# tdunnlab/scrubvae

Hardware: AMD Instinct MI355X
Metric: pose-windows/sec (ELBO-match) on synthetic 64-frame mouse skeletons (higher is better)
Workload: dtype f32 (f16x3b3 split on the fp16 / bf16 matrix cores); 1 GPU; configs[2] full SC-VAE (conditional + grad_reversal x2 + adversarial_net), AdamW, batch 4096/GPU, window 64, 23 joints, z=32, channels [64,128,256,512,1024]; batch_per_gpu=4096, global_batch=4096, window=64, joints=23, launch=eager launches, inputs=resident in HBM, side_streams=2, parallelism=dp1, backend=none, ranks_seen=1, bn=single rank

## Files before the change

scrubvae_amd/csrc/pose_tail.hip:

```cpp
#include "svae_internal.h"
#include <cstdlib>

namespace svae {

struct TailArgs {
  const float* y;
  const float* offsets;
  const float* target;
  const float* root;
  const float* ext_dx6d;
  const float* ext_droot;
  float* x6d_hat;
  float* root_hat;
  float* loss_part;
  float* dy;
  float* pose_out;
  long long rows;
  int ld, J, ldt, ldo;
  int has_arena;
  int pre_tanh;
  float a0[3], a1[3];
  float jpe_scale, root_scale;
  svae_tree tree;
};

struct M3 {
  float m[9];
};

__device__ __forceinline__ M3 mul(const M3& a, const M3& b) {
  M3 c;
#pragma unroll
  for (int r = 0; r < 3; ++r)
#pragma unroll
    for (int k = 0; k < 3; ++k) c.m[r * 3 + k] = a.m[r * 3] * b.m[k] + a.m[r * 3 + 1] * b.m[3 + k] + a.m[r * 3 + 2] * b.m[6 + k];
  return c;
}
__device__ __forceinline__ M3 mul_tn(const M3& a, const M3& b) {
  M3 c;
#pragma unroll
  for (int r = 0; r < 3; ++r)
#pragma unroll
    for (int k = 0; k < 3; ++k) c.m[r * 3 + k] = a.m[r] * b.m[k] + a.m[3 + r] * b.m[3 + k] + a.m[6 + r] * b.m[6 + k];
  return c;
}
__device__ __forceinline__ M3 mul_nt(const M3& a, const M3& b) {
  M3 c;
#pragma unroll
  for (int r = 0; r < 3; ++r)
#pragma unroll
    for (int k = 0; k < 3; ++k)
      c.m[r * 3 + k] = a.m[r * 3] * b.m[k * 3] + a.m[r * 3 + 1] * b.m[k * 3 + 1] + a.m[r * 3 + 2] * b.m[k * 3 + 2];
  return c;
}

__device__ __forceinline__ void cross3(const float* a, const float* b, float* c) {
  c[0] = a[1] * b[2] - a[2] * b[1];
  c[1] = a[2] * b[0] - a[0] * b[2];
  c[2] = a[0] * b[1] - a[1] * b[0];
}

constexpr float K1_EPS = 1e-8f;

__device__ __forceinline__ M3 c6_to_mat(const float* a) {
  const float nx = sqrtf(a[0] * a[0] + a[1] * a[1] + a[2] * a[2]);
  const float ix = 1.f / (nx + K1_EPS);
  const float x[3] = {a[0] * ix, a[1] * ix, a[2] * ix};
  float zr[3];
  cross3(x, a + 3, zr);
  const float nz = sqrtf(zr[0] * zr[0] + zr[1] * zr[1] + zr[2] * zr[2]);
  const float iz = 1.f / (nz + K1_EPS);
  const float z[3] = {zr[0] * iz, zr[1] * iz, zr[2] * iz};
  float yv[3];
  cross3(z, x, yv);
  M3 M;
#pragma unroll
  for (int r = 0; r < 3; ++r) { M.m[r * 3] = x[r]; M.m[r * 3 + 1] = yv[r]; M.m[r * 3 + 2] = z[r]; }
  return M;
}

__device__ __forceinline__ void c6_to_mat_bwd(const float* a, const M3& dM, float* da) {
  const float nx = sqrtf(a[0] * a[0] + a[1] * a[1] + a[2] * a[2]);
  const float ix = 1.f / (nx + K1_EPS);
  const float x[3] = {a[0] * ix, a[1] * ix, a[2] * ix};
  float zr[3];
  cross3(x, a + 3, zr);
  const float nz = sqrtf(zr[0] * zr[0] + zr[1] * zr[1] + zr[2] * zr[2]);
  const float iz = 1.f / (nz + K1_EPS);
  const float z[3] = {zr[0] * iz, zr[1] * iz, zr[2] * iz};
  float gx[3] = {dM.m[0], dM.m[3], dM.m[6]}, gy[3] = {dM.m[1], dM.m[4], dM.m[7]}, gz[3] = {dM.m[2], dM.m[5], dM.m[8]};
  float t[3];
  cross3(x, gy, t);
  gz[0] += t[0]; gz[1] += t[1]; gz[2] += t[2];
  cross3(gy, z, t);
  gx[0] += t[0]; gx[1] += t[1]; gx[2] += t[2];
  const float dzr_dot = zr[0] * gz[0] + zr[1] * gz[1] + zr[2] * gz[2];
  const float kz = nz > 0.f ? dzr_dot * iz * iz / nz : 0.f;
  const float gzr[3] = {gz[0] * iz - zr[0] * kz, gz[1] * iz - zr[1] * kz, gz[2] * iz - zr[2] * kz};
  cross3(a + 3, gzr, t);
  gx[0] += t[0]; gx[1] += t[1]; gx[2] += t[2];
  cross3(gzr, x, da + 3);
  const float dx_dot = a[0] * gx[0] + a[1] * gx[1] + a[2] * gx[2];
  const float kx = nx > 0.f ? dx_dot * ix * ix / nx : 0.f;
  da[0] = gx[0] * ix - a[0] * kx;
  da[1] = gx[1] * ix - a[1] * kx;
  da[2] = gx[2] * ix - a[2] * kx;
}

template <int TR>
__global__ __launch_bounds__(64 * SVAE_MAX_CHAINS) void pose_tail_kernel(const TailArgs g) {
  extern __shared__ __attribute__((aligned(16))) float smem[];
  const int tid = threadIdx.x, nth = blockDim.x;
  const int wave = tid >> 6, lane = tid & 63;
  const int J = g.J, J3 = 3 * J, C6 = 6 * J;
  const int ldt = g.ldt, ldo = g.ldo;
  float* tile = smem;
  float* offs = tile + TR * ldt;
  float* pose = offs + TR * ldo;
  float* dm0 = pose + TR * ldo;
  float* red = dm0 + TR * 9;
  const long long r0 = (long long)blockIdx.x * TR;
  const int nrows = (int)((g.rows - r0) < TR ? (g.rows - r0) : TR);
  const int n_chains = g.tree.n_chains;

  {
    const int f4_per_row = g.ld / 4;
    const int total = nrows * f4_per_row;
    const float* src = g.y + r0 * g.ld;
    for (int e = tid; e < total; e += nth) {
      const int rr = e / f4_per_row, c = (e - rr * f4_per_row) * 4;
      const float4 v = *reinterpret_cast<const float4*>(src + (long long)e * 4);
      float* d = tile + rr * ldt + c;
      if (g.pre_tanh) { d[0] = tanhf(v.x); d[1] = tanhf(v.y); d[2] = tanhf(v.z); d[3] = tanhf(v.w); }
      else { d[0] = v.x; d[1] = v.y; d[2] = v.z; d[3] = v.w; }
    }
    const int tot3 = nrows * J3;
    const float* so = g.offsets + r0 * J3;
    for (int e = tid; e < tot3; e += nth) {
      const int rr = e / J3, c = e - rr * J3;
      offs[rr * ldo + c] = so[e];
    }
    for (int e = tid; e < TR * 9; e += nth) dm0[e] = 0.f;
  }
  __syncthreads();
  {
    const int tot6 = nrows * C6;
    float* dst = g.x6d_hat + r0 * C6;
    for (int e = tid; e < tot6; e += nth) {
      const int rr = e / C6, c = e - rr * C6;
      dst[e] = tile[rr * ldt + c];
    }
    if (g.has_arena) {
      float* dr = g.root_hat + r0 * 3;
      for (int e = tid; e < nrows * 3; e += nth) {
        const int rr = e / 3, k = e - rr * 3;
        dr[e] = 0.5f * (tile[rr * ldt + C6 + k] + 1.f) * (g.a1[k] - g.a0[k]) + g.a0[k];
      }
    }
  }

  const bool active = lane < nrows;
  const int lrow = lane < TR ? lane : 0;
  float* my = tile + lrow * ldt;
  float* myo = offs + lrow * ldo;
  float* myp = pose + lrow * ldo;
  const bool do_bwd = g.dy != nullptr;
  const bool chain_wave = wave < n_chains && g.tree.chain_len[wave < n_chains ? wave : 0] >= 2;
  const int ch = wave < n_chains ? wave : 0;
  const int len = g.tree.chain_len[ch];

  float a6[6];
  M3 M0;
  if (active) {
#pragma unroll
    for (int k = 0; k < 6; ++k) a6[k] = my[k];
    M0 = c6_to_mat(a6);
  }
  M3 Rc = M0;
  if (active && chain_wave) {
    M3& R = Rc;
    float acc[3] = {0.f, 0.f, 0.f};
    for (int i = 1; i < len; ++i) {
      const int j = g.tree.chain[ch][i];
#pragma unroll
      for (int k = 0; k < 6; ++k) a6[k] = my[6 * j + k];
      R = mul(R, c6_to_mat(a6));
      const float o0 = myo[3 * j], o1 = myo[3 * j + 1], o2 = myo[3 * j + 2];
#pragma unroll
      for (int r = 0; r < 3; ++r) {
        acc[r] += R.m[r * 3] * o0 + R.m[r * 3 + 1] * o1 + R.m[r * 3 + 2] * o2;
        myp[3 * j + r] = acc[r];
      }
    }
  }
  __syncthreads();

  float rl = 0.f;
  if (wave == 0 && active) {
    myp[0] = 0.f; myp[1] = 0.f; myp[2] = 0.f;
    for (int c = 0; c < n_chains; ++c) {
      const int cl = g.tree.chain_len[c];
      const int head = g.tree.chain[c][0];
      const float h0 = myp[3 * head], h1 = myp[3 * head + 1], h2 = myp[3 * head + 2];
      for (int i = 1; i < cl; ++i) {
        const int j = g.tree.chain[c][i];
        myp[3 * j] += h0; myp[3 * j + 1] += h1; myp[3 * j + 2] += h2;
      }
    }
  }
  const int root_wave = nth > 64 ? 1 : 0;
  if (wave == root_wave && active && g.has_arena) {
#pragma unroll
    for (int k = 0; k < 3; ++k) {
      const float xh = my[C6 + k];
      const float half = 0.5f * (g.a1[k] - g.a0[k]);
      const float rh = (xh + 1.f) * half + g.a0[k];
      const float d = rh - g.root[(r0 + lane) * 3 + k];
      rl += d * d;
      if (do_bwd) {
        float gk = 2.f * g.root_scale * d;
        if (g.ext_droot) gk += g.ext_droot[(r0 + lane) * 3 + k];
        my[C6 + k] = g.pre_tanh ? gk * half * (1.f - xh * xh) : gk * half;
      }
    }
  }
  if (wave == root_wave && active && do_bwd) {
    for (int c = C6 + (g.has_arena ? 3 : 0); c < g.ld; ++c) my[c] = 0.f;
  }
  __syncthreads();

  {
    float jpe = 0.f;
    const int tot3 = nrows * J3;
    const float* stg = g.target + r0 * J3;
    float* dp = g.pose_out ? g.pose_out + r0 * J3 : nullptr;
    for (int e = tid; e < tot3; e += nth) {
      const int rr = e / J3, c = e - rr * J3;
      const float pv = pose[rr * ldo + c];
      if (dp) dp[e] = pv;
      const float d = pv - stg[e];
      jpe += d * d;
      pose[rr * ldo + c] = 2.f * g.jpe_scale * d;
    }
    jpe = wave_sum(jpe);
    if (lane == 0) red[wave] = jpe;
  }
  __syncthreads();
  if (tid == 0) {
    float t = 0.f;
    for (int w = 0; w < nth / 64; ++w) t += red[w];
    g.loss_part[blockIdx.x * 2] = t;
  }
  if (do_bwd && wave == 0 && active) {
    for (int c = n_chains - 1; c >= 0; --c) {
      const int cl = g.tree.chain_len[c];
      for (int i = cl - 1; i >= 1; --i) {
        const int j = g.tree.chain[c][i], par = g.tree.chain[c][i - 1];
#pragma unroll
        for (int r = 0; r < 3; ++r) myp[3 * par + r] += myp[3 * j + r];
      }
    }
  }
  if (do_bwd) __syncthreads();

  M3 carry;
#pragma unroll
  for (int k = 0; k < 9; ++k) carry.m[k] = 0.f;
  if (do_bwd && active && chain_wave) {
    M3 P = Rc;
#pragma unroll
    for (int i = SVAE_MAX_CHAIN_LEN - 1; i >= 1; --i) {
      if (i < len) {
        const int j = g.tree.chain[ch][i];
        M3 D = carry;
#pragma unroll
        for (int r = 0; r < 3; ++r)
#pragma unroll
          for (int k = 0; k < 3; ++k) D.m[r * 3 + k] += myp[3 * j + r] * myo[3 * j + k];
#pragma unroll
        for (int k = 0; k < 6; ++k) a6[k] = my[6 * j + k];
        const M3 Mj = c6_to_mat(a6);
        {
          float inv[3];
#pragma unroll
          for (int c = 0; c < 3; ++c) inv[c] = 1.f / (Mj.m[c] * Mj.m[c] + Mj.m[3 + c] * Mj.m[3 + c] + Mj.m[6 + c] * Mj.m[6 + c]);
          M3 Q;
#pragma unroll
          for (int r = 0; r < 3; ++r)
#pragma unroll
            for (int k = 0; k < 3; ++k)
              Q.m[r * 3 + k] = P.m[r * 3] * inv[0] * Mj.m[k * 3] + P.m[r * 3 + 1] * inv[1] * Mj.m[k * 3 + 1] + P.m[r * 3 + 2] * inv[2] * Mj.m[k * 3 + 2];
          P = Q;
        }
        const M3 dMj = mul_tn(P, D);
        carry = mul_nt(D, Mj);
        float da[6];
        c6_to_mat_bwd(a6, dMj, da);
#pragma unroll
        for (int k = 0; k < 6; ++k) {
          float gk = da[k];
          if (g.ext_dx6d) gk += g.ext_dx6d[(r0 + lane) * C6 + 6 * j + k];
          my[6 * j + k] = g.pre_tanh ? gk * (1.f - a6[k] * a6[k]) : gk;
        }
      }
    }
  }
  if (do_bwd) {
    for (int c = 0; c < n_chains; ++c) {
      if (wave == c && chain_wave && active) {
        float* d = dm0 + lane * 9;
#pragma unroll
        for (int k = 0; k < 9; ++k) d[k] += carry.m[k];
      }
      __syncthreads();
    }
  }
  if (do_bwd && wave == 0 && active) {
    M3 dM0;
    const float* d = dm0 + lane * 9;
#pragma unroll
    for (int k = 0; k < 9; ++k) dM0.m[k] = d[k];
    float a0[6], da0[6];
#pragma unroll
    for (int k = 0; k < 6; ++k) a0[k] = my[k];
    c6_to_mat_bwd(a0, dM0, da0);
#pragma unroll
    for (int k = 0; k < 6; ++k) {
      float gk = da0[k];
      if (g.ext_dx6d) gk += g.ext_dx6d[(r0 + lane) * C6 + k];
      my[k] = g.pre_tanh ? gk * (1.f - a0[k] * a0[k]) : gk;
    }
  }
  if (wave == root_wave) {
    rl = wave_sum(rl);
    if (lane == 0) g.loss_part[blockIdx.x * 2 + 1] = rl;
  }
  __syncthreads();
  if (do_bwd) {
    const int f4_per_row = g.ld / 4;
    const int total = nrows * f4_per_row;
    float* dst = g.dy + r0 * g.ld;
    for (int e = tid; e < total; e += nth) {
      const int rr = e / f4_per_row, c = (e - rr * f4_per_row) * 4;
      const float* sp = tile + rr * ldt + c;
      *reinterpret_cast<float4*>(dst + (long long)e * 4) = make_float4(sp[0], sp[1], sp[2], sp[3]);
    }
  }
}

__device__ __forceinline__ void rot6d_rows(const float* d6, float* m ) {
  const float n1 = fmaxf(sqrtf(d6[0] * d6[0] + d6[1] * d6[1] + d6[2] * d6[2]), 1e-12f);
  const float b1[3] = {d6[0] / n1, d6[1] / n1, d6[2] / n1};
  const float dt = b1[0] * d6[3] + b1[1] * d6[4] + b1[2] * d6[5];
  const float u[3] = {d6[3] - dt * b1[0], d6[4] - dt * b1[1], d6[5] - dt * b1[2]};
  const float n2 = fmaxf(sqrtf(u[0] * u[0] + u[1] * u[1] + u[2] * u[2]), 1e-12f);
  const float b2[3] = {u[0] / n2, u[1] / n2, u[2] / n2};
  float b3[3];
  cross3(b1, b2, b3);
#pragma unroll
  for (int k = 0; k < 3; ++k) { m[k] = b1[k]; m[3 + k] = b2[k]; m[6 + k] = b3[k]; }
}

__device__ __forceinline__ void rot6d_rows_bwd(const float* d6, const float* g, float* dd) {
  const float n1r = sqrtf(d6[0] * d6[0] + d6[1] * d6[1] + d6[2] * d6[2]);
  const float n1 = fmaxf(n1r, 1e-12f);
  const float b1[3] = {d6[0] / n1, d6[1] / n1, d6[2] / n1};
  const float dt = b1[0] * d6[3] + b1[1] * d6[4] + b1[2] * d6[5];
  const float u[3] = {d6[3] - dt * b1[0], d6[4] - dt * b1[1], d6[5] - dt * b1[2]};
  const float n2r = sqrtf(u[0] * u[0] + u[1] * u[1] + u[2] * u[2]);
  const float n2 = fmaxf(n2r, 1e-12f);
  const float b2[3] = {u[0] / n2, u[1] / n2, u[2] / n2};
  float gb1[3] = {g[0], g[1], g[2]}, gb2[3] = {g[3], g[4], g[5]};
  const float gb3[3] = {g[6], g[7], g[8]};
  float t[3];
  cross3(b2, gb3, t);
  gb1[0] += t[0]; gb1[1] += t[1]; gb1[2] += t[2];
  cross3(gb3, b1, t);
  gb2[0] += t[0]; gb2[1] += t[1]; gb2[2] += t[2];
  float gu[3];
  if (n2r > 1e-12f) {
    const float d = b2[0] * gb2[0] + b2[1] * gb2[1] + b2[2] * gb2[2];
#pragma unroll
    for (int k = 0; k < 3; ++k) gu[k] = (gb2[k] - b2[k] * d) / n2;
  } else {
#pragma unroll
    for (int k = 0; k < 3; ++k) gu[k] = gb2[k] / n2;
  }
  const float gub1 = gu[0] * b1[0] + gu[1] * b1[1] + gu[2] * b1[2];
#pragma unroll
  for (int k = 0; k < 3; ++k) {
    dd[3 + k] = gu[k] - gub1 * b1[k];
    gb1[k] += -dt * gu[k] - gub1 * d6[3 + k];
  }
  if (n1r > 1e-12f) {
    const float d = b1[0] * gb1[0] + b1[1] * gb1[1] + b1[2] * gb1[2];
#pragma unroll
    for (int k = 0; k < 3; ++k) dd[k] = (gb1[k] - b1[k] * d) / n1;
  } else {
#pragma unroll
    for (int k = 0; k < 3; ++k) dd[k] = gb1[k] / n1;
  }
}

__global__ __launch_bounds__(256) void rot_loss_kernel(const float* __restrict__ x, const float* __restrict__ xh, float scale,
                                                        float* __restrict__ part, float* __restrict__ dxh, long long n) {
  __shared__ float red4[4];
  const long long i = (long long)blockIdx.x * 256 + threadIdx.x;
  float loss = 0.f;
  if (i < n) {
    float a[6], b[6], m1[9], m2[9];
#pragma unroll
    for (int k = 0; k < 6; ++k) { a[k] = x[i * 6 + k]; b[k] = xh[i * 6 + k]; }
    rot6d_rows(a, m1);
    rot6d_rows(b, m2);
    float ss = 0.f, d[9];
#pragma unroll
    for (int k = 0; k < 9; ++k) { d[k] = m2[k] - m1[k]; ss += d[k] * d[k]; }
    const float fro = sqrtf(ss);
    const float c = 0.35355339059327373f;
    float s = fro * c;
    const float lim = 1.f - 1e-7f;
    const bool clamped = s > lim;
    if (clamped) s = lim;
    loss = 2.f * asinf(s);
    if (dxh) {
      float gm[9];
      const float gs = (!clamped && fro > 0.f) ? scale * 2.f / sqrtf(1.f - s * s) * c / fro : 0.f;
#pragma unroll
      for (int k = 0; k < 9; ++k) gm[k] = gs * d[k];
      float dd[6];
      rot6d_rows_bwd(b, gm, dd);
#pragma unroll
      for (int k = 0; k < 6; ++k) dxh[i * 6 + k] = dd[k];
    }
  }
  const float t = block_sum_256(loss, red4);
  if (threadIdx.x == 0) part[blockIdx.x] = t;
}

}

using namespace svae;

static int tail_rows() {
  static int tr = 0;
  if (tr == 0) {
    const char* e = getenv("SVAE_TAIL_ROWS");
    const int v = e ? atoi(e) : 64;
    tr = (v == 64 || v == 48 || v == 32) ? v : 64;
  }
  return tr;
}

extern "C" int svae_tail_blocks(long long rows) { const int tr = tail_rows(); return (int)((rows + tr - 1) / tr); }

extern "C" int svae_pose_tail(const float* y, int ld, const float* offsets, const float* target_pose, const float* root,
                              const float* arena_host, const svae_tree* tree, float jpe_scale, float root_scale,
                              const float* ext_dx6d, const float* ext_droot, float* x6d_hat, float* root_hat, float* loss_part,
                              float* dy, float* pose_out, long long rows, int input_is_pre_tanh, void* stream) {
  SVAE_REQUIRE(y && offsets && target_pose && tree && x6d_hat && loss_part && rows > 0, SVAE_ERR_ARG, "pose_tail: null pointer");
  const int J = tree->n_joints;
  SVAE_REQUIRE(J >= 1 && J <= SVAE_MAX_JOINTS && tree->n_chains >= 0 && tree->n_chains <= SVAE_MAX_CHAINS, SVAE_ERR_SHAPE,
               "pose_tail: bad tree");
  SVAE_REQUIRE(ld % 4 == 0 && ld >= 6 * J + (arena_host ? 3 : 0) && aligned16(y) && (!dy || aligned16(dy)), SVAE_ERR_ALIGN,
               "pose_tail: ld %d too small or misaligned", ld);
  SVAE_REQUIRE(!arena_host || (root && root_hat), SVAE_ERR_ARG, "pose_tail: arena without root buffers");
  int seen[SVAE_MAX_JOINTS] = {0};
  seen[0] = 1;
  for (int c = 0; c < tree->n_chains; ++c) {
    const int len = tree->chain_len[c];
    SVAE_REQUIRE(len >= 1 && len <= SVAE_MAX_CHAIN_LEN, SVAE_ERR_SHAPE, "pose_tail: chain %d length %d", c, len);
    for (int i = 0; i < len; ++i) SVAE_REQUIRE(tree->chain[c][i] >= 0 && tree->chain[c][i] < J, SVAE_ERR_SHAPE, "pose_tail: joint id");
    SVAE_REQUIRE(seen[tree->chain[c][0]], SVAE_ERR_SHAPE, "pose_tail: chain %d starts at a joint not yet placed", c);
    for (int i = 1; i < len; ++i) {
      SVAE_REQUIRE(!seen[tree->chain[c][i]], SVAE_ERR_SHAPE, "pose_tail: joint %d placed twice", tree->chain[c][i]);
      seen[tree->chain[c][i]] = 1;
    }
  }
  for (int j = 0; j < J; ++j) SVAE_REQUIRE(seen[j], SVAE_ERR_SHAPE, "pose_tail: joint %d not covered by the kinematic tree", j);
  TailArgs g;
  memset(&g, 0, sizeof(g));
  g.y = y; g.offsets = offsets; g.target = target_pose; g.root = root; g.ext_dx6d = ext_dx6d; g.ext_droot = ext_droot;
  g.x6d_hat = x6d_hat; g.root_hat = root_hat; g.loss_part = loss_part; g.dy = dy; g.pose_out = pose_out;
  g.rows = rows; g.ld = ld; g.J = J;
  g.ldt = ld | 1;
  g.ldo = (3 * J) | 1;
  g.has_arena = arena_host != nullptr;
  g.pre_tanh = input_is_pre_tanh;
  if (arena_host)
    for (int k = 0; k < 3; ++k) { g.a0[k] = arena_host[k]; g.a1[k] = arena_host[3 + k]; }
  g.jpe_scale = jpe_scale; g.root_scale = root_scale;
  g.tree = *tree;
  const int n_waves = tree->n_chains >= 2 ? tree->n_chains : 2;
  const int tr = tail_rows();
  const size_t smem = (size_t)(tr * g.ldt + 2 * tr * g.ldo + tr * 9 + SVAE_MAX_CHAINS) * sizeof(float);
  SVAE_REQUIRE(smem <= 160 * 1024, SVAE_ERR_SHAPE, "pose_tail: LDS tile %zu B exceeds 160 KiB", smem);
  static DeviceOnce attr_set;
  int attr_dev;
  if (attr_set.need(&attr_dev)) {
    hipError_t e = hipFuncSetAttribute((const void*)pose_tail_kernel<64>, hipFuncAttributeMaxDynamicSharedMemorySize, 160 * 1024);
    if (e == hipSuccess) e = hipFuncSetAttribute((const void*)pose_tail_kernel<48>, hipFuncAttributeMaxDynamicSharedMemorySize, 160 * 1024);
    if (e == hipSuccess) e = hipFuncSetAttribute((const void*)pose_tail_kernel<32>, hipFuncAttributeMaxDynamicSharedMemorySize, 160 * 1024);
    SVAE_REQUIRE(e == hipSuccess, SVAE_ERR_LAUNCH, "pose_tail: hipFuncSetAttribute(MaxDynamicSharedMemorySize): %s", hipGetErrorString(e));
    attr_set.done(attr_dev);
  }
  const dim3 grid(svae_tail_blocks(rows)), block(64 * n_waves);
  if (tr == 64) hipLaunchKernelGGL(pose_tail_kernel<64>, grid, block, smem, (hipStream_t)stream, g);
  else if (tr == 48) hipLaunchKernelGGL(pose_tail_kernel<48>, grid, block, smem, (hipStream_t)stream, g);
  else hipLaunchKernelGGL(pose_tail_kernel<32>, grid, block, smem, (hipStream_t)stream, g);
  return check_launch("pose_tail");
}

extern "C" int svae_rot_blocks(long long n) { return (int)((n + 255) / 256); }

extern "C" int svae_rot_loss(const float* x6d, const float* x6d_hat, float scale, float* part, float* dx6d_hat, long long n,
                             void* stream) {
  SVAE_REQUIRE(x6d && x6d_hat && part && n > 0, SVAE_ERR_ARG, "rot_loss: bad args");
  hipLaunchKernelGGL(rot_loss_kernel, dim3(svae_rot_blocks(n)), dim3(256), 0, (hipStream_t)stream, x6d, x6d_hat, scale, part,
                     dx6d_hat, n);
  return check_launch("rot_loss");
}
```

Before: 293,700 windows/s.

## Restructure pose tail kernel: precompute rotations, parallelize tree passes across threads

Rewrites the forward-kinematics tail so every thread in a larger block (up to 1024) converts 6D to rotation matrices per joint into an LDS buffer. Chain walks then reuse those matrices, and the serial per-row tree accumulation and backward scatter are spread across joint/row work items. The root-joint carry is reduced through LDS without a per-chain barrier loop. Global loads of offsets, targets and the external gradient are vectorized as float4 and issued early to hide latency. This adds LDS footprint and more barriers, drops the 48-row variant, and adds a denominator clamp in the backward pass.

Measured after the change: 294,900 windows/s, median of 3. Within noise of the previous version (+0.4%).

```diff
diff --git a/scrubvae_amd/csrc/pose_tail.hip b/scrubvae_amd/csrc/pose_tail.hip
--- a/scrubvae_amd/csrc/pose_tail.hip
+++ b/scrubvae_amd/csrc/pose_tail.hip
@@ -16,8 +16,9 @@
   float* dy;
   float* pose_out;
   long long rows;
-  int ld, J, ldt, ldo;
+  int ld, J, ldt, ldo, ldm;
   int has_arena;
+  int vec4;
   int pre_tanh;
   float a0[3], a1[3];
   float jpe_scale, root_scale;
@@ -107,183 +108,309 @@
   da[2] = gx[2] * ix - a[2] * kx;
 }
 
+__device__ __forceinline__ int row_of(int e, float inv) { return (int)(((float)e + 0.5f) * inv); }
+
 template <int TR>
-__global__ __launch_bounds__(64 * SVAE_MAX_CHAINS) void pose_tail_kernel(const TailArgs g) {
+__global__ __launch_bounds__(TR == 64 ? 1024 : 512) void pose_tail_kernel(const TailArgs g) {
   extern __shared__ __attribute__((aligned(16))) float smem[];
   const int tid = threadIdx.x, nth = blockDim.x;
   const int wave = tid >> 6, lane = tid & 63;
-  const int J = g.J, J3 = 3 * J, C6 = 6 * J;
-  const int ldt = g.ldt, ldo = g.ldo;
+  const int ldt = g.ldt, ldo = g.ldo, ldm = g.ldm;
+  const int n_chains = g.tree.n_chains;
   float* tile = smem;
   float* offs = tile + TR * ldt;
   float* pose = offs + TR * ldo;
-  float* dm0 = pose + TR * ldo;
-  float* red = dm0 + TR * 9;
-  const long long r0 = (long long)blockIdx.x * TR;
-  const int nrows = (int)((g.rows - r0) < TR ? (g.rows - r0) : TR);
-  const int n_chains = g.tree.n_chains;
-
-  {
+  float* rot = pose + TR * ldo;
+  float* car = rot + TR * ldm;
+  float* red = car + n_chains * TR * 9;
+  float* ebuf = offs;
+  constexpr int NY = TR == 64 ? 5 : 3, NU = TR == 64 ? 3 : 2, NE = TR == 64 ? 5 : 3;
+  const bool do_bwd = g.dy != nullptr;
+  const long long blk0 = (long long)blockIdx.x * 64;
+  const int cw = TR == 64 ? __builtin_amdgcn_readfirstlane(tid >> 6) : tid / TR;
+  const int cf = tid % TR;
+  const int ch = cw < n_chains ? cw : 0;
+  int* s_len = reinterpret_cast<int*>(red + 16);
+  int* s_chain = s_len + SVAE_MAX_CHAINS;
+  if (TR < 64) {
+    if (tid == 0)
+#pragma unroll 1
+      for (int c = 0; c < n_chains; ++c) {
+        s_len[c] = g.tree.chain_len[c];
+#pragma unroll 1
+        for (int i = 0; i < SVAE_MAX_CHAIN_LEN; ++i) s_chain[c * SVAE_MAX_CHAIN_LEN + i] = g.tree.chain[c][i];
+      }
+    __syncthreads();
+  }
+  auto chain_len = [&](int c) { return TR == 64 ? g.tree.chain_len[c] : s_len[c]; };
+  auto chain_joint = [&](int c, int i) { return TR == 64 ? g.tree.chain[c][i] : s_chain[c * SVAE_MAX_CHAIN_LEN + i]; };
+  const int len = n_chains ? chain_len(ch) : 0;
+  const bool has_chain = cw < n_chains && len >= 2;
+  const int root_wave = (nth >> 6) - 1;
+  float* myo = offs + cf * ldo;
+  float* myp = pose + cf * ldo;
+  float* myr = rot + cf * ldm;
+  float jpe_blk = 0.f, rl_blk = 0.f;
+
+  const int tid_blk = tid, nth_blk = nth;
+#pragma unroll 1
+  for (int sub = 0; sub < 64 / TR; ++sub) {
+    const long long r0 = blk0 + sub * TR;
+    if (r0 >= g.rows) break;
+    const int nrows = (int)((g.rows - r0) < TR ? (g.rows - r0) : TR);
+    if (sub) __syncthreads();
+    int tid = tid_blk, nth = nth_blk, J = g.J;
+    asm volatile("" : "+v"(tid), "+s"(nth), "+s"(J));
+    const int J3 = 3 * J, C6 = 6 * J, lde = C6 | 1;
     const int f4_per_row = g.ld / 4;
-    const int total = nrows * f4_per_row;
-    const float* src = g.y + r0 * g.ld;
-    for (int e = tid; e < total; e += nth) {
-      const int rr = e / f4_per_row, c = (e - rr * f4_per_row) * 4;
-      const float4 v = *reinterpret_cast<const float4*>(src + (long long)e * 4);
-      float* d = tile + rr * ldt + c;
-      if (g.pre_tanh) { d[0] = tanhf(v.x); d[1] = tanhf(v.y); d[2] = tanhf(v.z); d[3] = tanhf(v.w); }
-      else { d[0] = v.x; d[1] = v.y; d[2] = v.z; d[3] = v.w; }
-    }
-    const int tot3 = nrows * J3;
-    const float* so = g.offsets + r0 * J3;
-    for (int e = tid; e < tot3; e += nth) {
-      const int rr = e / J3, c = e - rr * J3;
-      offs[rr * ldo + c] = so[e];
-    }
-    for (int e = tid; e < TR * 9; e += nth) dm0[e] = 0.f;
-  }
-  __syncthreads();
-  {
-    const int tot6 = nrows * C6;
-    float* dst = g.x6d_hat + r0 * C6;
-    for (int e = tid; e < tot6; e += nth) {
-      const int rr = e / C6, c = e - rr * C6;
-      dst[e] = tile[rr * ldt + c];
-    }
-    if (g.has_arena) {
-      float* dr = g.root_hat + r0 * 3;
-      for (int e = tid; e < nrows * 3; e += nth) {
-        const int rr = e / 3, k = e - rr * 3;
-        dr[e] = 0.5f * (tile[rr * ldt + C6 + k] + 1.f) * (g.a1[k] - g.a0[k]) + g.a0[k];
-      }
-    }
-  }
-
-  const bool active = lane < nrows;
-  const int lrow = lane < TR ? lane : 0;
-  float* my = tile + lrow * ldt;
-  float* myo = offs + lrow * ldo;
-  float* myp = pose + lrow * ldo;
-  const bool do_bwd = g.dy != nullptr;
-  const bool chain_wave = wave < n_chains && g.tree.chain_len[wave < n_chains ? wave : 0] >= 2;
-  const int ch = wave < n_chains ? wave : 0;
-  const int len = g.tree.chain_len[ch];
-
-  float a6[6];
-  M3 M0;
-  if (active) {
-#pragma unroll
-    for (int k = 0; k < 6; ++k) a6[k] = my[k];
-    M0 = c6_to_mat(a6);
-  }
-  M3 Rc = M0;
-  if (active && chain_wave) {
-    M3& R = Rc;
-    float acc[3] = {0.f, 0.f, 0.f};
-    for (int i = 1; i < len; ++i) {
-      const int j = g.tree.chain[ch][i];
-#pragma unroll
-      for (int k = 0; k < 6; ++k) a6[k] = my[6 * j + k];
-      R = mul(R, c6_to_mat(a6));
-      const float o0 = myo[3 * j], o1 = myo[3 * j + 1], o2 = myo[3 * j + 2];
-#pragma unroll
-      for (int r = 0; r < 3; ++r) {
-        acc[r] += R.m[r * 3] * o0 + R.m[r * 3 + 1] * o1 + R.m[r * 3 + 2] * o2;
-        myp[3 * j + r] = acc[r];
-      }
-    }
-  }
-  __syncthreads();
-
-  float rl = 0.f;
-  if (wave == 0 && active) {
-    myp[0] = 0.f; myp[1] = 0.f; myp[2] = 0.f;
-    for (int c = 0; c < n_chains; ++c) {
-      const int cl = g.tree.chain_len[c];
-      const int head = g.tree.chain[c][0];
-      const float h0 = myp[3 * head], h1 = myp[3 * head + 1], h2 = myp[3 * head + 2];
-      for (int i = 1; i < cl; ++i) {
-        const int j = g.tree.chain[c][i];
-        myp[3 * j] += h0; myp[3 * j + 1] += h1; myp[3 * j + 2] += h2;
-      }
-    }
-  }
-  const int root_wave = nth > 64 ? 1 : 0;
-  if (wave == root_wave && active && g.has_arena) {
-#pragma unroll
-    for (int k = 0; k < 3; ++k) {
-      const float xh = my[C6 + k];
-      const float half = 0.5f * (g.a1[k] - g.a0[k]);
-      const float rh = (xh + 1.f) * half + g.a0[k];
-      const float d = rh - g.root[(r0 + lane) * 3 + k];
-      rl += d * d;
-      if (do_bwd) {
-        float gk = 2.f * g.root_scale * d;
-        if (g.ext_droot) gk += g.ext_droot[(r0 + lane) * 3 + k];
-        my[C6 + k] = g.pre_tanh ? gk * half * (1.f - xh * xh) : gk * half;
-      }
-    }
-  }
-  if (wave == root_wave && active && do_bwd) {
-    for (int c = C6 + (g.has_arena ? 3 : 0); c < g.ld; ++c) my[c] = 0.f;
-  }
-  __syncthreads();
-
-  {
-    float jpe = 0.f;
-    const int tot3 = nrows * J3;
+    const float inv_f4 = 1.f / (float)f4_per_row, inv_j3 = 1.f / (float)J3, inv_c6 = 1.f / (float)C6;
+    {
+      const int total = nrows * f4_per_row;
+      const int c_pad = C6 + (g.has_arena ? 3 : 0);
+      const float* src = g.y + r0 * g.ld;
+      const int tot3 = nrows * J3, n4 = g.vec4 ? tot3 / 4 : 0;
+      const float* so = g.offsets + r0 * J3;
+      float4 ov[NU];
+#pragma unroll
+      for (int u = 0; u < NU; ++u)
+        if (tid + u * nth < n4) ov[u] = reinterpret_cast<const float4*>(so)[tid + u * nth];
+      for (int e0 = tid; e0 < total; e0 += NY * nth) {
+        float4 yv[NY];
+#pragma unroll
+        for (int u = 0; u < NY; ++u)
+          if (e0 + u * nth < total) yv[u] = *reinterpret_cast<const float4*>(src + (long long)(e0 + u * nth) * 4);
+#pragma unroll
+        for (int u = 0; u < NY; ++u) {
+          const int e = e0 + u * nth;
+          if (e < total) {
+            const int rr = row_of(e, inv_f4), c = (e - rr * f4_per_row) * 4;
+            const float4 v = yv[u];
+            float* d = tile + rr * ldt + c;
+            if (g.pre_tanh && c < c_pad) { d[0] = tanhf(v.x); d[1] = tanhf(v.y); d[2] = tanhf(v.z); d[3] = tanhf(v.w); }
+            else { d[0] = v.x; d[1] = v.y; d[2] = v.z; d[3] = v.w; }
+          }
+        }
+      }
+#pragma unroll
+      for (int u = 0; u < NU; ++u) {
+        const int q = tid + u * nth;
+        if (q < n4) {
+          int rr = row_of(4 * q, inv_j3), c = 4 * q - rr * J3;
+          const float v[4] = {ov[u].x, ov[u].y, ov[u].z, ov[u].w};
+#pragma unroll
+          for (int k = 0; k < 4; ++k) {
+            offs[rr * ldo + c] = v[k];
+            if (++c == J3) { c = 0; ++rr; }
+          }
+        }
+      }
+      for (int e = (n4 > NU * nth ? NU * nth : n4) * 4 + tid; e < tot3; e += nth) {
+        const int rr = e / J3, c = e - rr * J3;
+        offs[rr * ldo + c] = so[e];
+      }
+    }
+    __syncthreads();
+    const int tot3 = nrows * J3, n4t = g.vec4 ? tot3 / 4 : 0;
     const float* stg = g.target + r0 * J3;
-    float* dp = g.pose_out ? g.pose_out + r0 * J3 : nullptr;
-    for (int e = tid; e < tot3; e += nth) {
-      const int rr = e / J3, c = e - rr * J3;
-      const float pv = pose[rr * ldo + c];
-      if (dp) dp[e] = pv;
-      const float d = pv - stg[e];
-      jpe += d * d;
-      pose[rr * ldo + c] = 2.f * g.jpe_scale * d;
-    }
-    jpe = wave_sum(jpe);
-    if (lane == 0) red[wave] = jpe;
-  }
-  __syncthreads();
-  if (tid == 0) {
-    float t = 0.f;
-    for (int w = 0; w < nth / 64; ++w) t += red[w];
-    g.loss_part[blockIdx.x * 2] = t;
-  }
-  if (do_bwd && wave == 0 && active) {
-    for (int c = n_chains - 1; c >= 0; --c) {
-      const int cl = g.tree.chain_len[c];
-      for (int i = cl - 1; i >= 1; --i) {
-        const int j = g.tree.chain[c][i], par = g.tree.chain[c][i - 1];
-#pragma unroll
-        for (int r = 0; r < 3; ++r) myp[3 * par + r] += myp[3 * j + r];
-      }
-    }
-  }
-  if (do_bwd) __syncthreads();
-
-  M3 carry;
-#pragma unroll
-  for (int k = 0; k < 9; ++k) carry.m[k] = 0.f;
-  if (do_bwd && active && chain_wave) {
-    M3 P = Rc;
-#pragma unroll
-    for (int i = SVAE_MAX_CHAIN_LEN - 1; i >= 1; --i) {
-      if (i < len) {
-        const int j = g.tree.chain[ch][i];
-        M3 D = carry;
+    float4 tv[NU];
+#pragma unroll
+    for (int u = 0; u < NU; ++u)
+      if (tid + u * nth < n4t) tv[u] = reinterpret_cast<const float4*>(stg)[tid + u * nth];
+    {
+      const int tot6 = nrows * C6, n4 = g.vec4 ? tot6 / 4 : 0;
+      float* dst = g.x6d_hat + r0 * C6;
+      for (int q = tid; q < n4; q += nth) {
+        int rr = row_of(4 * q, inv_c6), c = 4 * q - rr * C6;
+        float v[4];
+#pragma unroll
+        for (int k = 0; k < 4; ++k) {
+          v[k] = tile[rr * ldt + c];
+          if (++c == C6) { c = 0; ++rr; }
+        }
+        reinterpret_cast<float4*>(dst)[q] = make_float4(v[0], v[1], v[2], v[3]);
+      }
+      for (int e = n4 * 4 + tid; e < tot6; e += nth) {
+        const int rr = e / C6, c = e - rr * C6;
+        dst[e] = tile[rr * ldt + c];
+      }
+      if (g.has_arena) {
+        float* dr = g.root_hat + r0 * 3;
+        for (int e = tid; e < nrows * 3; e += nth) {
+          const int rr = e / 3, k = e - rr * 3;
+          dr[e] = 0.5f * (tile[rr * ldt + C6 + k] + 1.f) * (g.a1[k] - g.a0[k]) + g.a0[k];
+        }
+      }
+    }
+    for (int e = tid; e < J * TR; e += nth) {
+      const int f = e % TR, j = e / TR;
+      if (f < nrows) {
+        float a6[6];
+#pragma unroll
+        for (int k = 0; k < 6; ++k) a6[k] = tile[f * ldt + 6 * j + k];
+        const M3 M = c6_to_mat(a6);
+#pragma unroll
+        for (int k = 0; k < 9; ++k) rot[f * ldm + 9 * j + k] = M.m[k];
+      }
+    }
+    if (do_bwd) {
+      const int c0 = C6 + (g.has_arena ? 3 : 0), npad = g.ld - c0;
+      for (int e = tid; e < npad * TR; e += nth) {
+        const int f = e % TR, c = e / TR;
+        if (f < nrows) tile[f * ldt + c0 + c] = 0.f;
+      }
+    }
+    __syncthreads();
+
+    float rl = 0.f;
+    if (wave == root_wave && lane < nrows && g.has_arena) {
+      float* my = tile + lane * ldt;
+#pragma unroll
+      for (int k = 0; k < 3; ++k) {
+        const float xh = my[C6 + k];
+        const float half = 0.5f * (g.a1[k] - g.a0[k]);
+        const float rh = (xh + 1.f) * half + g.a0[k];
+        const float d = rh - g.root[(r0 + lane) * 3 + k];
+        rl += d * d;
+        if (do_bwd) {
+          float gk = 2.f * g.root_scale * d;
+          if (g.ext_droot) gk += g.ext_droot[(r0 + lane) * 3 + k];
+          my[C6 + k] = g.pre_tanh ? gk * half * (1.f - xh * xh) : gk * half;
+        }
+      }
+    }
+    if (wave == root_wave) {
+      rl = wave_sum(rl);
+      rl_blk += rl;
+    }
+    const bool citem = has_chain && cf < nrows;
+    M3 Rc;
+#pragma unroll
+    for (int k = 0; k < 9; ++k) Rc.m[k] = 0.f;
+    if (citem) {
+#pragma unroll
+      for (int k = 0; k < 9; ++k) Rc.m[k] = myr[k];
+      float acc[3] = {0.f, 0.f, 0.f};
+      for (int i = 1; i < len; ++i) {
+        const int j = chain_joint(ch, i);
+        M3 M;
+#pragma unroll
+        for (int k = 0; k < 9; ++k) M.m[k] = myr[9 * j + k];
+        Rc = mul(Rc, M);
+        const float o0 = myo[3 * j], o1 = myo[3 * j + 1], o2 = myo[3 * j + 2];
+#pragma unroll
+        for (int r = 0; r < 3; ++r) {
+          acc[r] += Rc.m[r * 3] * o0 + Rc.m[r * 3 + 1] * o1 + Rc.m[r * 3 + 2] * o2;
+          myp[3 * j + r] = acc[r];
+        }
+      }
+    }
+    __syncthreads();
+
+    for (int e = tid; e < 3 * TR; e += nth) {
+      const int f = e % TR;
+      if (f < nrows) {
+        float* p = pose + f * ldo + e / TR;
+        p[0] = 0.f;
+        for (int c = 0; c < n_chains; ++c) {
+          const int cl = chain_len(c);
+          const float h = p[3 * chain_joint(c, 0)];
+          float v[SVAE_MAX_CHAIN_LEN];
+#pragma unroll
+          for (int i = 1; i < SVAE_MAX_CHAIN_LEN; ++i)
+            if (i < cl) v[i] = p[3 * chain_joint(c, i)];
+#pragma unroll
+          for (int i = 1; i < SVAE_MAX_CHAIN_LEN; ++i)
+            if (i < cl) p[3 * chain_joint(c, i)] = v[i] + h;
+        }
+      }
+    }
+    __syncthreads();
+
+    {
+      float jpe = 0.f;
+      float* dp = g.pose_out ? g.pose_out + r0 * J3 : nullptr;
+#pragma unroll
+      for (int u = 0; u < NU; ++u) {
+        const int q = tid + u * nth;
+        if (q < n4t) {
+          int rr = row_of(4 * q, inv_j3), c = 4 * q - rr * J3;
+          const float t4[4] = {tv[u].x, tv[u].y, tv[u].z, tv[u].w};
+          float pv[4];
+#pragma unroll
+          for (int k = 0; k < 4; ++k) {
+            pv[k] = pose[rr * ldo + c];
+            const float d = pv[k] - t4[k];
+            jpe += d * d;
+            pose[rr * ldo + c] = 2.f * g.jpe_scale * d;
+            if (++c == J3) { c = 0; ++rr; }
+          }
+          if (dp) reinterpret_cast<float4*>(dp)[q] = make_float4(pv[0], pv[1], pv[2], pv[3]);
+        }
+      }
+      for (int e = (n4t > NU * nth ? NU * nth : n4t) * 4 + tid; e < tot3; e += nth) {
+        const int rr = e / J3, c = e - rr * J3;
+        const float pv = pose[rr * ldo + c];
+        if (dp) dp[e] = pv;
+        const float d = pv - stg[e];
+        jpe += d * d;
+        pose[rr * ldo + c] = 2.f * g.jpe_scale * d;
+      }
+      jpe = wave_sum(jpe);
+      if (lane == 0) red[wave] = jpe;
+    }
+    __syncthreads();
+    if (tid == 0) {
+      float t = 0.f;
+      for (int w = 0; w < nth / 64; ++w) t += red[w];
+      jpe_blk += t;
+    }
+    if (!do_bwd) continue;
+
+    for (int e = tid; e < 3 * TR; e += nth) {
+      const int f = e % TR;
+      if (f < nrows) {
+        float* p = pose + f * ldo + e / TR;
+        for (int c = n_chains - 1; c >= 0; --c) {
+          const int cl = chain_len(c);
+          float v[SVAE_MAX_CHAIN_LEN];
+#pragma unroll
+          for (int i = 0; i < SVAE_MAX_CHAIN_LEN; ++i)
+            if (i < cl) v[i] = p[3 * chain_joint(c, i)];
+#pragma unroll
+          for (int i = SVAE_MAX_CHAIN_LEN - 1; i >= 1; --i)
+            if (i < cl) {
+              v[i - 1] += v[i];
+              p[3 * chain_joint(c, i - 1)] = v[i - 1];
+            }
+        }
+      }
+    }
+    __syncthreads();
+
+    const int tot6 = nrows * C6, n4e = (g.ext_dx6d && g.vec4) ? tot6 / 4 : 0;
+    const float* se = g.ext_dx6d + r0 * C6;
+    float4 ev[NE];
+#pragma unroll
+    for (int u = 0; u < NE; ++u)
+      if (tid + u * nth < n4e) ev[u] = reinterpret_cast<const float4*>(se)[tid + u * nth];
+    if (citem) {
+      M3 carry, P = Rc;
+#pragma unroll
+      for (int k = 0; k < 9; ++k) carry.m[k] = 0.f;
+      for (int i = len - 1; i >= 1; --i) {
+        const int j = chain_joint(ch, i);
+        M3 D = carry, Mj;
+#pragma unroll
+        for (int k = 0; k < 9; ++k) Mj.m[k] = myr[9 * j + k];
 #pragma unroll
         for (int r = 0; r < 3; ++r)
 #pragma unroll
           for (int k = 0; k < 3; ++k) D.m[r * 3 + k] += myp[3 * j + r] * myo[3 * j + k];
-#pragma unroll
-        for (int k = 0; k < 6; ++k) a6[k] = my[6 * j + k];
-        const M3 Mj = c6_to_mat(a6);
         {
           float inv[3];
 #pragma unroll
-          for (int c = 0; c < 3; ++c) inv[c] = 1.f / (Mj.m[c] * Mj.m[c] + Mj.m[3 + c] * Mj.m[3 + c] + Mj.m[6 + c] * Mj.m[6 + c]);
+          for (int c = 0; c < 3; ++c)
+            inv[c] = 1.f / fmaxf(Mj.m[c] * Mj.m[c] + Mj.m[3 + c] * Mj.m[3 + c] + Mj.m[6 + c] * Mj.m[6 + c], 1e-30f);
           M3 Q;
 #pragma unroll
           for (int r = 0; r < 3; ++r)
@@ -294,58 +421,78 @@
         }
         const M3 dMj = mul_tn(P, D);
         carry = mul_nt(D, Mj);
-        float da[6];
-        c6_to_mat_bwd(a6, dMj, da);
+#pragma unroll
+        for (int k = 0; k < 9; ++k) myr[9 * j + k] = dMj.m[k];
+      }
+      float* d = car + (ch * TR + cf) * 9;
+#pragma unroll
+      for (int k = 0; k < 9; ++k) d[k] = carry.m[k];
+    }
+    __syncthreads();
+    if (g.ext_dx6d) {
+#pragma unroll
+      for (int u = 0; u < NE; ++u) {
+        const int q = tid + u * nth;
+        if (q < n4e) {
+          int rr = row_of(4 * q, inv_c6), c = 4 * q - rr * C6;
+          const float v[4] = {ev[u].x, ev[u].y, ev[u].z, ev[u].w};
+#pragma unroll
+          for (int k = 0; k < 4; ++k) {
+            ebuf[rr * lde + c] = v[k];
+            if (++c == C6) { c = 0; ++rr; }
+          }
+        }
+      }
+      for (int e = (n4e > NE * nth ? NE * nth : n4e) * 4 + tid; e < tot6; e += nth) {
+        const int rr = e / C6, c = e - rr * C6;
+        ebuf[rr * lde + c] = se[e];
+      }
+      __syncthreads();
+    }
+
+    for (int e = tid; e < J * TR; e += nth) {
+      const int f = e % TR, j = e / TR;
+      if (f < nrows) {
+        M3 dM;
+        if (j == 0) {
+#pragma unroll
+          for (int k = 0; k < 9; ++k) dM.m[k] = 0.f;
+          for (int c = 0; c < n_chains; ++c) {
+            if (chain_len(c) < 2) continue;
+            const float* d = car + (c * TR + f) * 9;
+#pragma unroll
+            for (int k = 0; k < 9; ++k) dM.m[k] += d[k];
+          }
+        } else {
+#pragma unroll
+          for (int k = 0; k < 9; ++k) dM.m[k] = rot[f * ldm + 9 * j + k];
+        }
+        float* my = tile + f * ldt + 6 * j;
+        float a6[6], da[6];
+#pragma unroll
+        for (int k = 0; k < 6; ++k) a6[k] = my[k];
+        c6_to_mat_bwd(a6, dM, da);
 #pragma unroll
         for (int k = 0; k < 6; ++k) {
           float gk = da[k];
-          if (g.ext_dx6d) gk += g.ext_dx6d[(r0 + lane) * C6 + 6 * j + k];
-          my[6 * j + k] = g.pre_tanh ? gk * (1.f - a6[k] * a6[k]) : gk;
-        }
-      }
-    }
-  }
-  if (do_bwd) {
-    for (int c = 0; c < n_chains; ++c) {
-      if (wave == c && chain_wave && active) {
-        float* d = dm0 + lane * 9;
-#pragma unroll
-        for (int k = 0; k < 9; ++k) d[k] += carry.m[k];
-      }
-      __syncthreads();
-    }
-  }
-  if (do_bwd && wave == 0 && active) {
-    M3 dM0;
-    const float* d = dm0 + lane * 9;
-#pragma unroll
-    for (int k = 0; k < 9; ++k) dM0.m[k] = d[k];
-    float a0[6], da0[6];
-#pragma unroll
-    for (int k = 0; k < 6; ++k) a0[k] = my[k];
-    c6_to_mat_bwd(a0, dM0, da0);
-#pragma unroll
-    for (int k = 0; k < 6; ++k) {
-      float gk = da0[k];
-      if (g.ext_dx6d) gk += g.ext_dx6d[(r0 + lane) * C6 + k];
-      my[k] = g.pre_tanh ? gk * (1.f - a0[k] * a0[k]) : gk;
-    }
-  }
-  if (wave == root_wave) {
-    rl = wave_sum(rl);
-    if (lane == 0) g.loss_part[blockIdx.x * 2 + 1] = rl;
-  }
-  __syncthreads();
-  if (do_bwd) {
-    const int f4_per_row = g.ld / 4;
-    const int total = nrows * f4_per_row;
-    float* dst = g.dy + r0 * g.ld;
-    for (int e = tid; e < total; e += nth) {
-      const int rr = e / f4_per_row, c = (e - rr * f4_per_row) * 4;
-      const float* sp = tile + rr * ldt + c;
-      *reinterpret_cast<float4*>(dst + (long long)e * 4) = make_float4(sp[0], sp[1], sp[2], sp[3]);
-    }
-  }
+          if (g.ext_dx6d) gk += ebuf[f * lde + 6 * j + k];
+          my[k] = g.pre_tanh ? gk * (1.f - a6[k] * a6[k]) : gk;
+        }
+      }
+    }
+    __syncthreads();
+    {
+      const int total = nrows * f4_per_row;
+      float* dst = g.dy + r0 * g.ld;
+      for (int e = tid; e < total; e += nth) {
+        const int rr = row_of(e, inv_f4), c = (e - rr * f4_per_row) * 4;
+        const float* sp = tile + rr * ldt + c;
+        *reinterpret_cast<float4*>(dst + (long long)e * 4) = make_float4(sp[0], sp[1], sp[2], sp[3]);
+      }
+    }
+  }
+  if (tid == 0) g.loss_part[blockIdx.x * 2] = jpe_blk;
+  if (wave == root_wave && lane == 0) g.loss_part[blockIdx.x * 2 + 1] = rl_blk;
 }
 
 __device__ __forceinline__ void rot6d_rows(const float* d6, float* m ) {
@@ -442,17 +589,17 @@
 
 using namespace svae;
 
-static int tail_rows() {
-  static int tr = 0;
-  if (tr == 0) {
-    const char* e = getenv("SVAE_TAIL_ROWS");
-    const int v = e ? atoi(e) : 64;
-    tr = (v == 64 || v == 48 || v == 32) ? v : 64;
-  }
-  return tr;
-}
-
-extern "C" int svae_tail_blocks(long long rows) { const int tr = tail_rows(); return (int)((rows + tr - 1) / tr); }
+static size_t tail_lds(int tr, const svae::TailArgs& g) {
+  return (size_t)(tr * (g.ldt + 2 * g.ldo + g.ldm + 9 * g.tree.n_chains) + 16 + SVAE_MAX_CHAINS * (1 + SVAE_MAX_CHAIN_LEN)) * sizeof(float);
+}
+
+static int tail_env(const char* name, int a, int b, int c) {
+  const char* e = getenv(name);
+  const int v = e ? atoi(e) : 0;
+  return (v == a || v == b || v == c) ? v : 0;
+}
+
+extern "C" int svae_tail_blocks(long long rows) { return (int)((rows + 63) / 64); }
 
 extern "C" int svae_pose_tail(const float* y, int ld, const float* offsets, const float* target_pose, const float* root,
                               const float* arena_host, const svae_tree* tree, float jpe_scale, float root_scale,
@@ -484,29 +631,32 @@
   g.x6d_hat = x6d_hat; g.root_hat = root_hat; g.loss_part = loss_part; g.dy = dy; g.pose_out = pose_out;
   g.rows = rows; g.ld = ld; g.J = J;
   g.ldt = ld | 1;
-  g.ldo = (3 * J) | 1;
+  g.ldo = (3 * J + 1) | 1;
+  g.ldm = (9 * J) | 1;
   g.has_arena = arena_host != nullptr;
+  g.vec4 = aligned16(offsets) && aligned16(target_pose) && (!pose_out || aligned16(pose_out)) && (!ext_dx6d || aligned16(ext_dx6d)) && aligned16(x6d_hat);
   g.pre_tanh = input_is_pre_tanh;
   if (arena_host)
     for (int k = 0; k < 3; ++k) { g.a0[k] = arena_host[k]; g.a1[k] = arena_host[3 + k]; }
   g.jpe_scale = jpe_scale; g.root_scale = root_scale;
   g.tree = *tree;
-  const int n_waves = tree->n_chains >= 2 ? tree->n_chains : 2;
-  const int tr = tail_rows();
-  const size_t smem = (size_t)(tr * g.ldt + 2 * tr * g.ldo + tr * 9 + SVAE_MAX_CHAINS) * sizeof(float);
+  static const int env_tr = tail_env("SVAE_TAIL_ROWS", 64, 32, 32), env_nt = tail_env("SVAE_TAIL_THREADS", 256, 512, 1024);
+  const int tr = env_tr ? env_tr : (tail_lds(64, g) <= 160 * 1024 ? 64 : 32);
+  const size_t smem = tail_lds(tr, g);
   SVAE_REQUIRE(smem <= 160 * 1024, SVAE_ERR_SHAPE, "pose_tail: LDS tile %zu B exceeds 160 KiB", smem);
+  const int chain_threads = (tree->n_chains * tr + 63) / 64 * 64, base_threads = env_nt ? env_nt : (tr == 64 ? 1024 : 512);
+  int threads = chain_threads > base_threads ? chain_threads : base_threads;
+  if (tr != 64 && threads > 512) threads = 512;
   static DeviceOnce attr_set;
   int attr_dev;
   if (attr_set.need(&attr_dev)) {
     hipError_t e = hipFuncSetAttribute((const void*)pose_tail_kernel<64>, hipFuncAttributeMaxDynamicSharedMemorySize, 160 * 1024);
-    if (e == hipSuccess) e = hipFuncSetAttribute((const void*)pose_tail_kernel<48>, hipFuncAttributeMaxDynamicSharedMemorySize, 160 * 1024);
     if (e == hipSuccess) e = hipFuncSetAttribute((const void*)pose_tail_kernel<32>, hipFuncAttributeMaxDynamicSharedMemorySize, 160 * 1024);
     SVAE_REQUIRE(e == hipSuccess, SVAE_ERR_LAUNCH, "pose_tail: hipFuncSetAttribute(MaxDynamicSharedMemorySize): %s", hipGetErrorString(e));
     attr_set.done(attr_dev);
   }
-  const dim3 grid(svae_tail_blocks(rows)), block(64 * n_waves);
+  const dim3 grid(svae_tail_blocks(rows)), block(threads);
   if (tr == 64) hipLaunchKernelGGL(pose_tail_kernel<64>, grid, block, smem, (hipStream_t)stream, g);
-  else if (tr == 48) hipLaunchKernelGGL(pose_tail_kernel<48>, grid, block, smem, (hipStream_t)stream, g);
   else hipLaunchKernelGGL(pose_tail_kernel<32>, grid, block, smem, (hipStream_t)stream, g);
   return check_launch("pose_tail");
 }
```
